# zhang-tao-whu/DVIS_Plus

Hardware: AMD Instinct MI355X
Metric: frames/sec DVIS++ R50 offline, 720p T=30 synthetic (higher is better)
Workload: dtype f32 (storage, accumulation, results; the segmenter's dense layers - R50 convolutions from 128 channels on, pixel-decoder projections and FPN output convolution, the deformable encoder's projections and FFN, the decoder's key / value projections - multiply each fp32 operand as two f16 terms on the f1

## Files before the change

dvis_plus_amd/csrc/gemm.hip:

```cpp
#include "dvis_common.h"

namespace {

constexpr unsigned kOOB = 0x80000000u;

struct GemmArgs {
  const float *A, *W, *bias, *res;
  float *C;
  long long lda, ldw, ldres, ldc;
  long long sA, sW, sRes, sC, sBias;
  int M, N, K, act, row_blocks, col_blocks, vec_store, col_fastest;
};

template <int TILES> constexpr int kGemmMinWaves = TILES >= 32 ? 1 : (TILES >= 20 ? 2 : (TILES >= 12 ? 3 : 4));

template <int RT, int CT, int NW, int PF, bool K16>
__global__ __launch_bounds__(64 * NW, kGemmMinWaves<RT * CT>) void gemm_nt_kernel(const GemmArgs p) {
  extern __shared__ float lds[];
  constexpr int BM = 16 * RT, BN = 16 * CT, T = 64 * NW;

  const int tid = threadIdx.x, lane = tid & 63;
  const int wv = __builtin_amdgcn_readfirstlane(tid >> 6);
  const int i = lane & 15, g = lane >> 4;
  int rb, cb;
  if (p.col_fastest) {
    const unsigned tiles = gridDim.x, xcd = blockIdx.x & 7u, slot = blockIdx.x >> 3;
    const unsigned q8 = tiles >> 3, r8 = tiles & 7u;
    const unsigned logical = (xcd < r8 ? xcd * (q8 + 1) : r8 * (q8 + 1) + (xcd - r8) * q8) + slot;
    rb = (int)(logical / (unsigned)p.col_blocks), cb = (int)(logical % (unsigned)p.col_blocks);
  } else {
    rb = blockIdx.x % p.row_blocks, cb = blockIdx.x / p.row_blocks;
  }
  const int row0 = rb * BM, col0 = cb * BN;
  const long long batch = blockIdx.y;

  const int rows_a = min(BM, p.M - row0), rows_w = min(BN, p.N - col0);
  const float *Ab = p.A + batch * p.sA + (long long)row0 * p.lda;
  const float *Wb = p.W + batch * p.sW + (long long)col0 * p.ldw;
  const __amdgpu_buffer_rsrc_t ra = dvis_make_rsrc_uniform(Ab, (unsigned)((((long long)rows_a - 1) * p.lda + p.K) * 4));
  const __amdgpu_buffer_rsrc_t rw = dvis_make_rsrc_uniform(Wb, (unsigned)((((long long)rows_w - 1) * p.ldw + p.K) * 4));
  unsigned aoff[RT], woff[CT];
#pragma unroll
  for (int rt = 0; rt < RT; ++rt) aoff[rt] = (unsigned)((rt * 16 + i) * p.lda * 4 + g * 16);
#pragma unroll
  for (int ct = 0; ct < CT; ++ct) woff[ct] = (unsigned)((ct * 16 + i) * p.ldw * 4 + g * 16);

  const int G = (p.K + 15) >> 4;
  const int g0 = (int)((long long)G * wv / NW), g1 = (int)((long long)G * (wv + 1) / NW);

  dvis_f4 a[PF][RT], w[PF][CT];
  auto load = [&](int slot, int grp) {
    const bool in = grp < g1;
    const unsigned so = in ? (unsigned)grp * 64u : 0u;
    const bool kv = in && (K16 || grp * 16 + g * 4 < p.K);
#pragma unroll
    for (int rt = 0; rt < RT; ++rt)
      a[slot][rt] = __builtin_bit_cast(
          dvis_f4, __builtin_amdgcn_raw_buffer_load_b128(ra, kv ? aoff[rt] : kOOB, so, 0));
#pragma unroll
    for (int ct = 0; ct < CT; ++ct)
      w[slot][ct] = __builtin_bit_cast(
          dvis_f4, __builtin_amdgcn_raw_buffer_load_b128(rw, kv ? woff[ct] : kOOB, so, 0));
  };

  dvis_f4 acc[RT][CT];
#pragma unroll
  for (int rt = 0; rt < RT; ++rt)
#pragma unroll
    for (int ct = 0; ct < CT; ++ct) acc[rt][ct] = dvis_f4{0.f, 0.f, 0.f, 0.f};

  auto contract = [&](int s) {
#pragma unroll
    for (int c = 0; c < 4; ++c)
#pragma unroll
      for (int rt = 0; rt < RT; ++rt)
#pragma unroll
        for (int ct = 0; ct < CT; ++ct)
          acc[rt][ct] = __builtin_amdgcn_mfma_f32_16x16x4f32(a[s][rt][c], w[s][ct][c], acc[rt][ct], 0, 0, 0);
  };
#pragma unroll
  for (int s = 0; s < PF; ++s) load(s, g0 + s);
  int grp = g0;
#pragma unroll 1
  for (; grp + 2 * PF <= g1; grp += PF) {
#pragma unroll
    for (int s = 0; s < PF; ++s) {
      contract(s);
      __builtin_amdgcn_sched_barrier(0);
      load(s, grp + s + PF);
      __builtin_amdgcn_sched_barrier(0);
    }
  }
  if (grp + PF <= g1) {
#pragma unroll
    for (int s = 0; s < PF; ++s) {
      contract(s);
      if (grp + s + PF < g1) load(s, grp + s + PF);
    }
    grp += PF;
  }
#pragma unroll
  for (int s = 0; s < PF; ++s)
    if (grp + s < g1) contract(s);

  float *mine = lds + wv * (BM * BN);
#pragma unroll
  for (int rt = 0; rt < RT; ++rt)
#pragma unroll
    for (int ct = 0; ct < CT; ++ct)
#pragma unroll
      for (int r = 0; r < 4; ++r) mine[(rt * 16 + g * 4 + r) * BN + ct * 16 + i] = acc[rt][ct][r];
  __syncthreads();

  constexpr int U = BM * BN / 4, UR = BN / 4;
  float *Cb = p.C + batch * p.sC;
  const float *Rb = p.res ? p.res + batch * p.sRes : nullptr;
  const float *Bb = p.bias ? p.bias + batch * p.sBias : nullptr;
#pragma unroll
  for (int u0 = 0; u0 < U; u0 += T) {
    const int u = u0 + tid;
    if (U % T != 0 && u >= U) break;
    const int row = u / UR, c4 = (u - row * UR) * 4;
    dvis_f4 s = *reinterpret_cast<const dvis_f4 *>(lds + row * BN + c4);
#pragma unroll
    for (int k = 1; k < NW; ++k) {
      const dvis_f4 t = *reinterpret_cast<const dvis_f4 *>(lds + k * (BM * BN) + row * BN + c4);
      s = dvis_f4{s[0] + t[0], s[1] + t[1], s[2] + t[2], s[3] + t[3]};
    }
    const int gr = row0 + row, gc = col0 + c4;
    if (gr >= p.M || gc >= p.N) continue;
    float *dst = Cb + (long long)gr * p.ldc + gc;
    if (p.vec_store) {
      if (Bb) {
        const dvis_f4 b = *reinterpret_cast<const dvis_f4 *>(Bb + gc);
        s = dvis_f4{s[0] + b[0], s[1] + b[1], s[2] + b[2], s[3] + b[3]};
      }
      if (Rb) {
        const dvis_f4 t = *reinterpret_cast<const dvis_f4 *>(Rb + (long long)gr * p.ldres + gc);
        s = dvis_f4{s[0] + t[0], s[1] + t[1], s[2] + t[2], s[3] + t[3]};
      }
      if (p.act) s = dvis_f4{fmaxf(s[0], 0.f), fmaxf(s[1], 0.f), fmaxf(s[2], 0.f), fmaxf(s[3], 0.f)};
      *reinterpret_cast<dvis_f4 *>(dst) = s;
    } else {
#pragma unroll
      for (int e = 0; e < 4; ++e) {
        if (gc + e >= p.N) break;
        float v = s[e];
        if (Bb) v += Bb[gc + e];
        if (Rb) v += Rb[(long long)gr * p.ldres + gc + e];
        if (p.act) v = fmaxf(v, 0.f);
        dst[e] = v;
      }
    }
  }
}

template <int RT, int CT, int PF, bool K16>
__global__ __launch_bounds__(64, kGemmMinWaves<RT * CT>) void gemm_nt_persist_kernel(const GemmArgs p) {
  extern __shared__ float lds[];
  constexpr int BM = 16 * RT, BN = 16 * CT, T = 64;
  const int tid = threadIdx.x, lane = tid;
  const int i = lane & 15, g = lane >> 4;
  const long long total = (long long)p.row_blocks * p.col_blocks;
  const unsigned gsz = gridDim.x;
  long long t = (long long)(blockIdx.x & 7u) * (gsz >> 3) + (blockIdx.x >> 3);
  const long long batch = blockIdx.y;
  const float *A0 = p.A + batch * p.sA, *W0 = p.W + batch * p.sW;
  unsigned aoff[RT], woff[CT];
#pragma unroll
  for (int rt = 0; rt < RT; ++rt) aoff[rt] = (unsigned)((rt * 16 + i) * p.lda * 4 + g * 16);
#pragma unroll
  for (int ct = 0; ct < CT; ++ct) woff[ct] = (unsigned)((ct * 16 + i) * p.ldw * 4 + g * 16);
  const int g1 = (p.K + 15) >> 4;

  int row0 = (int)(t / p.col_blocks) * BM, col0 = (int)(t % p.col_blocks) * BN;
  auto desc_a = [&](int r0) {
    const int rows = min(BM, p.M - r0);
    return dvis_make_rsrc_uniform(A0 + (long long)r0 * p.lda, (unsigned)((((long long)rows - 1) * p.lda + p.K) * 4));
  };
  auto desc_w = [&](int c0) {
    const int rows = min(BN, p.N - c0);
    return dvis_make_rsrc_uniform(W0 + (long long)c0 * p.ldw, (unsigned)((((long long)rows - 1) * p.ldw + p.K) * 4));
  };
  __amdgpu_buffer_rsrc_t ra = desc_a(row0), rw = desc_w(col0);

  dvis_f4 a[PF][RT], w[PF][CT];
  auto load = [&](int slot, int grp) {
    const bool in = grp < g1;
    const unsigned so = in ? (unsigned)grp * 64u : 0u;
    const bool kv = in && (K16 || grp * 16 + g * 4 < p.K);
#pragma unroll
    for (int rt = 0; rt < RT; ++rt)
      a[slot][rt] = __builtin_bit_cast(dvis_f4, __builtin_amdgcn_raw_buffer_load_b128(ra, kv ? aoff[rt] : kOOB, so, 0));
#pragma unroll
    for (int ct = 0; ct < CT; ++ct)
      w[slot][ct] = __builtin_bit_cast(dvis_f4, __builtin_amdgcn_raw_buffer_load_b128(rw, kv ? woff[ct] : kOOB, so, 0));
  };
  dvis_f4 acc[RT][CT];
  auto contract = [&](int s) {
#pragma unroll
    for (int c = 0; c < 4; ++c)
#pragma unroll
      for (int rt = 0; rt < RT; ++rt)
#pragma unroll
        for (int ct = 0; ct < CT; ++ct)
          acc[rt][ct] = __builtin_amdgcn_mfma_f32_16x16x4f32(a[s][rt][c], w[s][ct][c], acc[rt][ct], 0, 0, 0);
  };
#pragma unroll
  for (int s = 0; s < PF; ++s) load(s, s);

  float *Cb = p.C + batch * p.sC;
  const float *Rb = p.res ? p.res + batch * p.sRes : nullptr;
  const __amdgpu_buffer_rsrc_t rbias =
      dvis_make_rsrc_uniform(p.bias ? p.bias + batch * p.sBias : p.A, p.bias ? (unsigned)p.N * 4u : 0u);
#pragma unroll 1
  for (;;) {
#pragma unroll
    for (int rt = 0; rt < RT; ++rt)
#pragma unroll
      for (int ct = 0; ct < CT; ++ct) acc[rt][ct] = dvis_f4{0.f, 0.f, 0.f, 0.f};
    int grp = 0;
    auto round = [&]() {
#pragma unroll
      for (int s = 0; s < PF; ++s) {
        contract(s);
        __builtin_amdgcn_sched_barrier(0);
        load(s, grp + s + PF);
        __builtin_amdgcn_sched_barrier(0);
      }
      grp += PF;
    };
    if (grp + 2 * PF <= g1) round();
#pragma unroll 1
    while (grp + 2 * PF <= g1) round();
    if (grp + PF <= g1) {
#pragma unroll
      for (int s = 0; s < PF; ++s) {
        contract(s);
        if (grp + s + PF < g1) load(s, grp + s + PF);
      }
      grp += PF;
    }
#pragma unroll
    for (int s = 0; s < PF; ++s)
      if (grp + s < g1) contract(s);

    const long long tn = t + gsz;
    const bool more = tn < total;
    const int row_e = row0, col_e = col0;
    static_assert(T % (BN / 4) == 0, "a thread keeps its column quad over the epilogue's rounds");
    const int c4_mine = (tid % (BN / 4)) * 4;
    const dvis_f4 bias4 = __builtin_bit_cast(
        dvis_f4, __builtin_amdgcn_raw_buffer_load_b128(rbias, (unsigned)(col_e + c4_mine) * 4u, 0, 0));
    if (more) {
      row0 = (int)(tn / p.col_blocks) * BM, col0 = (int)(tn % p.col_blocks) * BN;
      ra = desc_a(row0), rw = desc_w(col0);
#pragma unroll
      for (int s = 0; s < PF; ++s) load(s, s);
    }
    __syncthreads();
#pragma unroll
    for (int rt = 0; rt < RT; ++rt)
#pragma unroll
      for (int ct = 0; ct < CT; ++ct)
#pragma unroll
        for (int r = 0; r < 4; ++r) lds[(rt * 16 + g * 4 + r) * BN + ct * 16 + i] = acc[rt][ct][r];
    __syncthreads();
    constexpr int U = BM * BN / 4, UR = BN / 4;
#pragma unroll 4
    for (int u = tid; u < U; u += T) {
      const int row = u / UR, c4 = (u - row * UR) * 4;
      dvis_f4 sv = *reinterpret_cast<const dvis_f4 *>(lds + row * BN + c4);
      const int gr = row_e + row, gc = col_e + c4;
      if (gr >= p.M || gc >= p.N) continue;
      float *dst = Cb + (long long)gr * p.ldc + gc;
      if (p.vec_store) {
        sv = dvis_f4{sv[0] + bias4[0], sv[1] + bias4[1], sv[2] + bias4[2], sv[3] + bias4[3]};
        if (Rb) {
          const dvis_f4 tq = *reinterpret_cast<const dvis_f4 *>(Rb + (long long)gr * p.ldres + gc);
          sv = dvis_f4{sv[0] + tq[0], sv[1] + tq[1], sv[2] + tq[2], sv[3] + tq[3]};
        }
        if (p.act) sv = dvis_f4{fmaxf(sv[0], 0.f), fmaxf(sv[1], 0.f), fmaxf(sv[2], 0.f), fmaxf(sv[3], 0.f)};
        *reinterpret_cast<dvis_f4 *>(dst) = sv;
      } else {
#pragma unroll
        for (int e = 0; e < 4; ++e) {
          if (gc + e >= p.N) break;
          float v = sv[e] + bias4[e];
          if (Rb) v += Rb[(long long)gr * p.ldres + gc + e];
          if (p.act) v = fmaxf(v, 0.f);
          dst[e] = v;
        }
      }
    }
    if (!more) break;
    t = tn;
  }
}

struct Config {
  int rt, ct, nw;
  void (*kernel16)(const GemmArgs);
  void (*kernel4)(const GemmArgs);
  void (*persist16)(const GemmArgs);
  void (*persist4)(const GemmArgs);
};
template <int RT, int CT, int NW, int PF, bool K16> constexpr auto persist_or_null() -> void (*)(const GemmArgs) {
  if constexpr (NW == 1) return gemm_nt_persist_kernel<RT, CT, PF, K16>;
  else return nullptr;
}

#define DVIS_GEMM_CFG(RT_, CT_, NW_, PF_)                                                                      \
  { RT_, CT_, NW_, gemm_nt_kernel<RT_, CT_, NW_, PF_, true>, gemm_nt_kernel<RT_, CT_, NW_, PF_, false>,            \
    persist_or_null<RT_, CT_, NW_, PF_, true>(), persist_or_null<RT_, CT_, NW_, PF_, false>() }
const Config kConfigs[] = {
    DVIS_GEMM_CFG(1, 1, 4, 4),
    DVIS_GEMM_CFG(1, 1, 8, 4),
    DVIS_GEMM_CFG(2, 1, 8, 4),
    DVIS_GEMM_CFG(2, 2, 4, 4),
    DVIS_GEMM_CFG(2, 2, 8, 2),
    DVIS_GEMM_CFG(4, 1, 8, 4),
    DVIS_GEMM_CFG(4, 2, 4, 2),
    DVIS_GEMM_CFG(4, 2, 8, 2),
    DVIS_GEMM_CFG(4, 4, 4, 2),
    DVIS_GEMM_CFG(4, 4, 2, 2),
    DVIS_GEMM_CFG(7, 1, 8, 2),
    DVIS_GEMM_CFG(7, 2, 4, 2),
    DVIS_GEMM_CFG(4, 4, 1, 2),
    DVIS_GEMM_CFG(8, 4, 2, 2),
    DVIS_GEMM_CFG(8, 4, 1, 2),
    DVIS_GEMM_CFG(6, 4, 1, 2),
    DVIS_GEMM_CFG(5, 4, 1, 2),
};
constexpr int kNumConfigs = sizeof(kConfigs) / sizeof(kConfigs[0]);

int pick_config(int M, int N, int K, int batch) {
  auto wgs = [&](int c) {
    const long long rb = (M + 16 * kConfigs[c].rt - 1) / (16 * kConfigs[c].rt);
    const long long cb = (N + 16 * kConfigs[c].ct - 1) / (16 * kConfigs[c].ct);
    return rb * cb * batch;
  };
  if ((long long)M * K * 4 > (64ll << 20) && N >= 64) return 14;
  if (wgs(8) >= 256 || (K >= 1024 && wgs(8) >= 128)) return 8;
  if (wgs(6) >= 256) return 6;
  if (wgs(3) >= 192) return K >= 1024 ? 4 : 3;
  if (wgs(2) >= 96) return 2;
  return K >= 256 ? 1 : 0;
}

int pick_config_nw(int M, int N, int K, int batch, int nw) {
  auto wgs = [&](int c) {
    const long long rb = (M + 16 * kConfigs[c].rt - 1) / (16 * kConfigs[c].rt);
    const long long cb = (N + 16 * kConfigs[c].ct - 1) / (16 * kConfigs[c].ct);
    return rb * cb * batch;
  };
  if (nw == 1) return ((long long)M * K * 4 > (64ll << 20) && N >= 64) || wgs(14) >= 1024 ? 14 : 12;
  if (nw == 4) {
    if (wgs(8) >= 256 || (K >= 1024 && wgs(8) >= 128)) return 8;
    if (wgs(6) >= 256) return 6;
    if (wgs(3) >= 192) return 3;
    return 0;
  }
  if (wgs(7) >= 256) return 7;
  if (wgs(4) >= 192) return 4;
  if (wgs(2) >= 96) return 2;
  return 1;
}

}

DVIS_EXPORT int dvis_gemm_num_configs(void) { return kNumConfigs; }

DVIS_EXPORT int dvis_gemm_pick_config_nw(int M, int N, int K, int batch, int nw) {
  if (nw != 1 && nw != 4 && nw != 8) return -1;
  return pick_config_nw(M, N, K, batch > 0 ? batch : 1, nw);
}

DVIS_EXPORT int dvis_gemm_config_waves(int config) { return config >= 0 && config < kNumConfigs ? kConfigs[config].nw : -1; }

DVIS_EXPORT int dvis_gemm_pick_config(int M, int N, int K, int batch) { return pick_config(M, N, K, batch > 0 ? batch : 1); }

static int gemm_launch(const float *A, int64_t lda, int64_t strideA, const float *W, int64_t ldw, int64_t strideW,
                       const float *bias, int64_t strideBias, const float *res, int64_t ldres, int64_t strideRes, float *C,
                       int64_t ldc, int64_t strideC, int M, int N, int K, int batch, int act, int config, void *stream) {
  DVIS_REQUIRE(M >= 0 && N >= 0 && K > 0 && batch >= 0, "gemm_nt: bad sizes (M=%d N=%d K=%d batch=%d)", M, N, K, batch);
  if (M == 0 || N == 0 || batch == 0) return DVIS_OK;
  DVIS_REQUIRE(A && W && C, "gemm_nt: null pointer");
  DVIS_REQUIRE(K % 4 == 0 && lda % 4 == 0 && ldw % 4 == 0 && strideA % 4 == 0 && strideW % 4 == 0 &&
                   ((uintptr_t)A | (uintptr_t)W) % 16 == 0,
               "gemm_nt: needs K, lda, ldw, batch strides %% 4 == 0 and 16-byte aligned A / W (K=%d lda=%lld ldw=%lld)", K,
               (long long)lda, (long long)ldw);
  DVIS_REQUIRE(lda >= K && ldw >= K && ldc >= N && (!res || ldres >= N),
               "gemm_nt: row strides shorter than the rows");
  DVIS_REQUIRE(batch <= 65535, "gemm_nt: batch <= 65535");
  const int c = config >= 0 ? config : pick_config(M, N, K, batch);
  DVIS_REQUIRE(c < kNumConfigs, "gemm_nt: configuration %d does not exist", c);
  const Config &cf = kConfigs[c];
  const int BM = 16 * cf.rt, BN = 16 * cf.ct;
  DVIS_REQUIRE((long long)BM * lda * 4 < (1ll << 31) && (long long)BN * ldw * 4 < (1ll << 31),
               "gemm_nt: one tile's rows must span less than 2 GiB");
  GemmArgs p;
  p.A = A, p.W = W, p.bias = bias, p.res = res, p.C = C;
  p.lda = lda, p.ldw = ldw, p.ldres = ldres, p.ldc = ldc;
  p.sA = strideA, p.sW = strideW, p.sRes = strideRes, p.sC = strideC, p.sBias = strideBias;
  p.M = M, p.N = N, p.K = K, p.act = act;
  p.row_blocks = (M + BM - 1) / BM;
  p.col_blocks = (N + BN - 1) / BN;
  p.col_fastest = (long long)M * K * 4 > (64ll << 20) && p.col_blocks > 1;
  p.vec_store = N % 4 == 0 && ldc % 4 == 0 && strideC % 4 == 0 && (uintptr_t)C % 16 == 0 &&
                (!bias || ((uintptr_t)bias % 16 == 0 && strideBias % 4 == 0)) &&
                (!res || (ldres % 4 == 0 && strideRes % 4 == 0 && (uintptr_t)res % 16 == 0));
  const long long tiles = (long long)p.row_blocks * p.col_blocks;
  DVIS_REQUIRE(tiles < (1ll << 31), "gemm_nt: too many tiles");
  const size_t lds = (size_t)cf.nw * BM * BN * sizeof(float);
  auto kernel = K % 16 == 0 ? cf.kernel16 : cf.kernel4;
  static DvisLdsOptIn opted[kNumConfigs][2];
  if (const int rc = dvis_lds_opt_in(reinterpret_cast<const void *>(kernel), lds, &opted[c][K % 16 == 0 ? 0 : 1], "gemm_nt"))
    return rc;
  static const bool persist_on = []() { const char *e = getenv("DVIS_GEMM_PERSIST"); return !(e && e[0] == '0'); }();
  auto pk = K % 16 == 0 ? cf.persist16 : cf.persist4;
  if (persist_on && pk != nullptr && p.col_fastest) {
    static int cus = 0;
    if (cus == 0) {
      int dev = 0, n = 0;
      hipGetDevice(&dev);
      cus = hipDeviceGetAttribute(&n, hipDeviceAttributeMultiprocessorCount, dev) == hipSuccess && n > 0 ? n : 256;
    }
    const int tiles_cnt = cf.rt * cf.ct;
    const int occ = tiles_cnt >= 32 ? 1 : (tiles_cnt >= 20 ? 2 : (tiles_cnt >= 12 ? 3 : 4));
    const size_t lds1 = (size_t)BM * BN * sizeof(float);
    long long per_cu = 4ll * occ;
    if ((long long)(160 * 1024 / lds1) < per_cu) per_cu = (long long)(160 * 1024 / lds1);
    long long grid = (long long)cus * per_cu;
    if (grid > tiles) grid = tiles;
    grid &= ~7ll;
    if (grid >= 8) {
      hipLaunchKernelGGL(pk, dim3((unsigned)grid, (unsigned)batch), dim3(64), lds1, (hipStream_t)stream, p);
      return dvis_check_launch("gemm_nt_persist_kernel");
    }
  }
  hipLaunchKernelGGL(kernel, dim3((unsigned)tiles, (unsigned)batch), dim3(64 * cf.nw), lds, (hipStream_t)stream, p);
  return dvis_check_launch("gemm_nt_kernel");
}

DVIS_EXPORT int dvis_gemm_nt(const float *A, int64_t lda, int64_t strideA, const float *W, int64_t ldw, int64_t strideW,
                             const float *bias, const float *res, int64_t ldres, int64_t strideRes, float *C,
                             int64_t ldc, int64_t strideC, int M, int N, int K, int batch, int act, int config,
                             void *stream) {
  return gemm_launch(A, lda, strideA, W, ldw, strideW, bias, 0, res, ldres, strideRes, C, ldc, strideC, M, N, K, batch, act,
                     config, stream);
}

DVIS_EXPORT int dvis_gemm_nt_bb(const float *A, int64_t lda, int64_t strideA, const float *W, int64_t ldw, int64_t strideW,
                                const float *bias, int64_t strideBias, const float *res, int64_t ldres, int64_t strideRes,
                                float *C, int64_t ldc, int64_t strideC, int M, int N, int K, int batch, int act, int config,
                                void *stream) {
  return gemm_launch(A, lda, strideA, W, ldw, strideW, bias, strideBias, res, ldres, strideRes, C, ldc, strideC, M, N, K,
                     batch, act, config, stream);
}
```

dvis_plus_amd/csrc/postprocess.hip:

```cpp
#include <math.h>

#include "dvis_common.h"
#include "torch_cpu_math.h"

namespace {

constexpr int kMaxK = 256;
using tcpu::Geometry;
using tcpu::Tap;

__global__ __launch_bounds__(256) void vps_argmax_kernel(
    const float *__restrict__ logits, int64_t stride_k, int64_t stride_t, const float *__restrict__ scores, int K, int T,
    int h, int w, int first_h, int first_w, int img_h, int img_w, int out_h, int out_w, int *__restrict__ ids,
    uint8_t *__restrict__ conf, int *__restrict__ areas ) {
  __shared__ int s_area[3 * kMaxK];
  for (int i = threadIdx.x; i < 3 * K; i += 256) s_area[i] = 0;
  __syncthreads();

  const size_t npix = (size_t)T * out_h * out_w;
  const Geometry g(h, w, first_h, first_w, img_h, img_w, out_h, out_w);
  const int lane = threadIdx.x & 63;
  for (size_t base = (size_t)blockIdx.x * 256; base < npix; base += (size_t)gridDim.x * 256) {
    const size_t p = base + threadIdx.x;
    const bool valid = p < npix;
    const size_t pc = valid ? p : npix - 1;
    const int X = (int)(pc % out_w);
    const size_t r = pc / out_w;
    const int Y = (int)(r % out_h);
    const int t = (int)(r / out_h);
    const Tap ty = tcpu::make_tap(Y, g.s2y, img_h, out_h), tx = tcpu::make_tap(X, g.s2x, img_w, out_w);
    const int kind1 = tcpu::bilinear_kind(first_h, first_w, t, T), kind2 = tcpu::bilinear_kind(out_h, out_w, t, T);
    float best = -INFINITY, best_prob = 0.f;
    int best_k = 0;
    for (int k = 0; k < K; ++k) {
      const float *lg = logits + (size_t)k * stride_k + (size_t)t * stride_t;
      const float prob = tcpu::two_stage<true>(lg, g, Y, X, ty, tx, kind1, kind2);
      const unsigned long long over = __ballot(valid && prob >= 0.5f);
      if (lane == 0 && over) atomicAdd(&s_area[K + k], __popcll(over));
      const float sc = scores[k] * prob;
      if (sc > best) {
        best = sc;
        best_k = k;
        best_prob = prob;
      }
    }
    if (valid) {
      const bool cf = best_prob >= 0.5f;
      ids[p] = best_k;
      conf[p] = cf ? 1 : 0;
      atomicAdd(&s_area[best_k], 1);
      if (cf) atomicAdd(&s_area[2 * K + best_k], 1);
    }
  }
  __syncthreads();
  for (int i = threadIdx.x; i < 3 * K; i += 256)
    if (s_area[i]) atomicAdd(&areas[i], s_area[i]);
}

template <int K4>
__global__ __launch_bounds__(256) void vss_argmax_kernel(
    const float *__restrict__ logits, int64_t stride_q, int64_t stride_t, const float *__restrict__ cls, int Q, int C, int T,
    int h, int w, int first_h, int first_w, int img_h, int img_w, int out_h, int out_w, int64_t *__restrict__ out) {
  const size_t npix = (size_t)T * out_h * out_w;
  const Geometry g(h, w, first_h, first_w, img_h, img_w, out_h, out_w);
  const bool identity2 = img_h == out_h && img_w == out_w;
  for (size_t base = (size_t)blockIdx.x * 256; base < npix; base += (size_t)gridDim.x * 256) {
    const size_t p = base + threadIdx.x;
    const bool valid = p < npix;
    const size_t pc = valid ? p : npix - 1;
    const int X = (int)(pc % out_w);
    const size_t r = pc / out_w;
    const int Y = (int)(r % out_h);
    const int t = (int)(r / out_h);
    const Tap ty = tcpu::make_tap(Y, g.s2y, img_h, out_h), tx = tcpu::make_tap(X, g.s2x, img_w, out_w);
    const int kind1 = tcpu::bilinear_kind(first_h, first_w, t, T), kind2 = tcpu::bilinear_kind(out_h, out_w, t, T);
    float4 acc[K4];
#pragma unroll
    for (int k = 0; k < K4; ++k) acc[k] = make_float4(0.f, 0.f, 0.f, 0.f);
    auto accumulate = [&](int q, float prob) {
      const float4 *row = reinterpret_cast<const float4 *>(cls + (size_t)q * 4 * K4);
#pragma unroll
      for (int k = 0; k < K4; ++k) {
        const float4 cv = row[k];
        acc[k].x += cv.x * prob; acc[k].y += cv.y * prob; acc[k].z += cv.z * prob; acc[k].w += cv.w * prob;
      }
    };
    if (identity2) {
      const Tap sy = tcpu::make_tap(Y, g.s1y, h, first_h), sx = tcpu::make_tap(X, g.s1x, w, first_w);
      const int o00 = sy.i0 * w + sx.i0, o01 = sy.i0 * w + sx.i1, o10 = sy.i1 * w + sx.i0, o11 = sy.i1 * w + sx.i1;
      const float *lg = logits + (size_t)t * stride_t;
      const bool tail = X >= g.tail_x;
      float a = lg[o00], b = lg[o01], c = lg[o10], d = lg[o11];
#pragma unroll 1
      for (int q = 0; q < Q; ++q) {
        const float v = tcpu::bilinear(a, b, c, d, sy, sx, kind1);
        if (q + 1 < Q) {
          const float *nx = lg + (size_t)(q + 1) * stride_q;
          a = nx[o00]; b = nx[o01]; c = nx[o10]; d = nx[o11];
        }
        accumulate(q, tcpu::sigmoid(v, tail));
      }
    } else {
#pragma unroll 1
      for (int q = 0; q < Q; ++q) {
        const float *lg = logits + (size_t)q * stride_q + (size_t)t * stride_t;
        accumulate(q, tcpu::two_stage<true>(lg, g, Y, X, ty, tx, kind1, kind2));
      }
    }
    float best = -INFINITY;
    int best_c = 0;
#pragma unroll
    for (int k = 0; k < K4; ++k) {
      if (4 * k < C && acc[k].x > best) { best = acc[k].x; best_c = 4 * k; }
      if (4 * k + 1 < C && acc[k].y > best) { best = acc[k].y; best_c = 4 * k + 1; }
      if (4 * k + 2 < C && acc[k].z > best) { best = acc[k].z; best_c = 4 * k + 2; }
      if (4 * k + 3 < C && acc[k].w > best) { best = acc[k].w; best_c = 4 * k + 3; }
    }
    if (valid) out[p] = best_c;
  }
}

__global__ __launch_bounds__(256) void vss_argmax_mfma_kernel(
    const float *__restrict__ logits, int64_t stride_q, int64_t stride_t, const float *__restrict__ cls ,
    int Q, int Qp, int C, int T, int h, int w, int first_h, int first_w, int out_h, int out_w, int64_t *__restrict__ out) {
  extern __shared__ __attribute__((aligned(16))) float s_cls[];
  constexpr int LSC = 132;
  constexpr int NT = 2;
  for (int i = threadIdx.x; i < Qp * 128; i += 256) s_cls[(i >> 7) * LSC + (i & 127)] = cls[i];
  __syncthreads();
  const int lane = threadIdx.x & 63, wv = threadIdx.x >> 6;
  const int j = lane & 15, gq = lane >> 4;
  const size_t npix = (size_t)T * out_h * out_w;
  const Geometry g(h, w, first_h, first_w, out_h, out_w, out_h, out_w);
  const size_t nchunks = (npix + 16 * NT - 1) / (16 * NT);
  for (size_t chunk = (size_t)blockIdx.x * 4 + wv; chunk < nchunks; chunk += (size_t)gridDim.x * 4) {
    const float *l00[NT], *l01[NT], *l10[NT], *l11[NT];
    Tap ty1[NT], tx1[NT];
    int kind1[NT];
    bool tail[NT];
#pragma unroll
    for (int n = 0; n < NT; ++n) {
      const size_t p = min(chunk * (16 * NT) + (size_t)n * 16 + j, npix - 1);
      const int X = (int)(p % out_w);
      const size_t r = p / out_w;
      const int Y = (int)(r % out_h);
      const Tap sy = tcpu::make_tap(Y, g.s1y, h, first_h), sx = tcpu::make_tap(X, g.s1x, w, first_w);
      const float *base = logits + (size_t)(r / out_h) * stride_t + (size_t)gq * stride_q;
      l00[n] = base + sy.i0 * w + sx.i0; l01[n] = base + sy.i0 * w + sx.i1;
      l10[n] = base + sy.i1 * w + sx.i0; l11[n] = base + sy.i1 * w + sx.i1;
      ty1[n] = sy; tx1[n] = sx;
      kind1[n] = tcpu::bilinear_kind(first_h, first_w, (int)(r / out_h), T);
      tail[n] = X >= g.tail_x;
    }
    dvis_f4 acc[8][NT];
#pragma unroll
    for (int mt = 0; mt < 8; ++mt)
#pragma unroll
      for (int n = 0; n < NT; ++n) acc[mt][n] = dvis_f4{0.f, 0.f, 0.f, 0.f};
    float va[NT], vb[NT], vc[NT], vd[NT];
    const size_t step = (size_t)4 * stride_q;
#pragma unroll
    for (int n = 0; n < NT; ++n) { va[n] = *l00[n]; vb[n] = *l01[n]; vc[n] = *l10[n]; vd[n] = *l11[n]; }
#pragma unroll 1
    for (int ks = 0; ks < Qp; ks += 4) {
      float pb[NT];
#pragma unroll
      for (int n = 0; n < NT; ++n) {
        pb[n] = tcpu::sigmoid(tcpu::bilinear(va[n], vb[n], vc[n], vd[n], ty1[n], tx1[n], kind1[n]), tail[n]);
      }
      if (ks + 4 < Qp) {
#pragma unroll
        for (int n = 0; n < NT; ++n) {
          l00[n] += step; l01[n] += step; l10[n] += step; l11[n] += step;
          va[n] = *l00[n]; vb[n] = *l01[n]; vc[n] = *l10[n]; vd[n] = *l11[n];
        }
      }
      const float *arow = s_cls + (size_t)(ks + gq) * LSC + j;
#pragma unroll
      for (int mt = 0; mt < 8; ++mt) {
        const float a = arow[16 * mt];
#pragma unroll
        for (int n = 0; n < NT; ++n) acc[mt][n] = __builtin_amdgcn_mfma_f32_16x16x4f32(a, pb[n], acc[mt][n], 0, 0, 0);
      }
    }
#pragma unroll
    for (int n = 0; n < NT; ++n) {
      float best = -INFINITY;
      int best_c = 0x7fffffff;
#pragma unroll
      for (int mt = 0; mt < 8; ++mt)
#pragma unroll
        for (int r = 0; r < 4; ++r) {
          const int c = 16 * mt + 4 * gq + r;
          const float v = acc[mt][n][r];
          if (c < C && v > best) { best = v; best_c = c; }
        }
#pragma unroll
      for (int o = 16; o <= 32; o <<= 1) {
        const float ov = __shfl_xor(best, o);
        const int oc = __shfl_xor(best_c, o);
        if (ov > best || (ov == best && oc < best_c)) { best = ov; best_c = oc; }
      }
      const size_t p = chunk * (16 * NT) + (size_t)n * 16 + j;
      if (gq == 0 && p < npix) out[p] = best_c;
    }
  }
}

__global__ __launch_bounds__(256) void resize2_gt0_kernel(
    const float *__restrict__ logits, int64_t stride_k, int64_t stride_t, int K, int T, int h, int w, int first_h,
    int first_w, int img_h, int img_w, int out_h, int out_w, uint8_t *__restrict__ out) {
  const Geometry g(h, w, first_h, first_w, img_h, img_w, out_h, out_w);
  const int wq = (out_w + 3) >> 2;
  const size_t ngroups = (size_t)K * T * out_h * wq;
  const bool word_ok = (out_w & 3) == 0;
  for (size_t gi = (size_t)blockIdx.x * 256 + threadIdx.x; gi < ngroups; gi += (size_t)gridDim.x * 256) {
    const int xg = (int)(gi % wq);
    size_t r = gi / wq;
    const int Y = (int)(r % out_h);
    r /= out_h;
    const int t = (int)(r % T);
    const int k = (int)(r / T);
    const float *lg = logits + (size_t)k * stride_k + (size_t)t * stride_t;
    const Tap ty = tcpu::make_tap(Y, g.s2y, img_h, out_h);
    const int kind1 = tcpu::bilinear_kind(first_h, first_w, t, T), kind2 = tcpu::bilinear_kind(out_h, out_w, t, T);
    uint8_t *orow = out + (((size_t)k * T + t) * out_h + Y) * out_w;
    unsigned word = 0;
#pragma unroll
    for (int i = 0; i < 4; ++i) {
      const int X = 4 * xg + i;
      if (X < out_w) {
        const Tap tx = tcpu::make_tap(X, g.s2x, img_w, out_w);
        const bool on = tcpu::two_stage<false>(lg, g, Y, X, ty, tx, kind1, kind2) > 0.f;
        if (word_ok) word |= (on ? 1u : 0u) << (8 * i);
        else orow[X] = on ? 1 : 0;
      }
    }
    if (word_ok) *reinterpret_cast<unsigned *>(orow + 4 * xg) = word;
  }
}

template <bool SIGMOID>
__global__ __launch_bounds__(256) void resize2_kernel(
    const float *__restrict__ logits, int64_t stride_k, int64_t stride_t, int K, int T, int h, int w, int first_h,
    int first_w, int img_h, int img_w, int out_h, int out_w, float *__restrict__ out) {
  const Geometry g(h, w, first_h, first_w, img_h, img_w, out_h, out_w);
  const size_t npix = (size_t)K * T * out_h * out_w;
  for (size_t p = (size_t)blockIdx.x * 256 + threadIdx.x; p < npix; p += (size_t)gridDim.x * 256) {
    const int X = (int)(p % out_w);
    size_t r = p / out_w;
    const int Y = (int)(r % out_h);
    r /= out_h;
    const int t = (int)(r % T);
    const int k = (int)(r / T);
    const Tap ty = tcpu::make_tap(Y, g.s2y, img_h, out_h), tx = tcpu::make_tap(X, g.s2x, img_w, out_w);
    const int kind1 = tcpu::bilinear_kind(first_h, first_w, t, T), kind2 = tcpu::bilinear_kind(out_h, out_w, t, T);
    out[p] = tcpu::two_stage<SIGMOID>(logits + (size_t)k * stride_k + (size_t)t * stride_t, g, Y, X, ty, tx, kind1, kind2);
  }
}

}

DVIS_EXPORT int dvis_vps_argmax(const float *logits, int64_t stride_k, int64_t stride_t, const float *scores, int K, int T,
                                int h, int w, int first_h, int first_w, int img_h, int img_w, int out_h, int out_w,
                                int32_t *ids, uint8_t *conf, int32_t *areas, void *stream) {
  DVIS_REQUIRE(K > 0 && K <= kMaxK && T >= 0 && h > 0 && w > 0 && first_h > 0 && first_w > 0 && img_h > 0 && img_w > 0 &&
                   out_h > 0 && out_w > 0,
               "vps_argmax: bad sizes (K must be 1..%d)", kMaxK);
  DVIS_REQUIRE(img_h <= first_h && img_w <= first_w, "vps_argmax: image size exceeds the padded size");
  DVIS_REQUIRE((size_t)T * out_h * out_w < 0x7fffffffu, "vps_argmax: more than 2^31 output pixels");
  DVIS_REQUIRE(logits && scores && ids && conf && areas, "vps_argmax: null pointer");
  hipStream_t st = (hipStream_t)stream;
  if (const int rc = dvis_zero_words(areas, (size_t)3 * K, st, "vps_argmax: zero areas")) return rc;
  if (T == 0) return DVIS_OK;
  const size_t npix = (size_t)T * out_h * out_w;
  size_t blocks = (npix + 255) / 256;
  if (blocks > 256 * 16) blocks = 256 * 16;
  hipLaunchKernelGGL(vps_argmax_kernel, dim3((unsigned)blocks), dim3(256), 0, st, logits, stride_k, stride_t, scores, K, T,
                     h, w, first_h, first_w, img_h, img_w, out_h, out_w, ids, conf, areas);
  return dvis_check_launch("vps_argmax_kernel");
}

DVIS_EXPORT int dvis_vss_argmax(const float *logits, int64_t stride_q, int64_t stride_t, const float *cls,
                                int cls_row_stride, int Q, int C, int T, int h, int w, int first_h, int first_w, int img_h, int img_w, int out_h, int out_w,
                                int64_t *out, void *stream) {
  DVIS_REQUIRE(Q > 0 && C > 0 && C <= 128 && T >= 0 && h > 0 && w > 0 && first_h > 0 && first_w > 0 && img_h > 0 &&
                   img_w > 0 && out_h > 0 && out_w > 0,
               "vss_argmax: bad sizes (C must be 1..128)");
  DVIS_REQUIRE(img_h <= first_h && img_w <= first_w, "vss_argmax: image size exceeds the padded size");
  DVIS_REQUIRE(logits && cls && out, "vss_argmax: null pointer");
  if (T == 0) return DVIS_OK;
  DVIS_REQUIRE(cls_row_stride >= C && cls_row_stride % 32 == 0 && cls_row_stride <= 128 && (((uintptr_t)cls) & 15) == 0,
               "vss_argmax: cls rows must be zero padded to a multiple of 32 floats (<= 128), 16-byte aligned");
  const int k4 = cls_row_stride / 4;
  hipStream_t st = (hipStream_t)stream;
  const size_t npix = (size_t)T * out_h * out_w;
  size_t blocks = (npix + 255) / 256;
  if (img_h == out_h && img_w == out_w && cls_row_stride == 128 && Q % 4 == 0) {
    const size_t lds = (size_t)Q * 132 * sizeof(float);
    if (lds <= 64 * 1024) {
      size_t nb = ((npix + 31) / 32 + 3) / 4;
      if (nb > 256 * 9) nb = 256 * 9;
      hipLaunchKernelGGL(vss_argmax_mfma_kernel, dim3((unsigned)nb), dim3(256), lds, st, logits, stride_q, stride_t, cls, Q, Q,
                         C, T, h, w, first_h, first_w, out_h, out_w, out);
      return dvis_check_launch("vss_argmax_mfma_kernel");
    }
  }
  if (blocks > 256 * 16) blocks = 256 * 16;
#define DVIS_VSS(K4_)                                                                                                   \
  hipLaunchKernelGGL((vss_argmax_kernel<K4_>), dim3((unsigned)blocks), dim3(256), 0, st, logits, stride_q, stride_t, cls, \
                     Q, C, T, h, w, first_h, first_w, img_h, img_w, out_h, out_w, out)
  if (k4 == 8) DVIS_VSS(8);
  else if (k4 == 16) DVIS_VSS(16);
  else if (k4 == 24) DVIS_VSS(24);
  else DVIS_VSS(32);
#undef DVIS_VSS
  return dvis_check_launch("vss_argmax_kernel");
}

DVIS_EXPORT int dvis_resize2_gt0(const float *logits, int64_t stride_k, int64_t stride_t, int K, int T, int h, int w,
                                 int first_h, int first_w, int img_h, int img_w, int out_h, int out_w, uint8_t *out,
                                 void *stream) {
  DVIS_REQUIRE(K >= 0 && T >= 0 && h > 0 && w > 0 && first_h > 0 && first_w > 0 && img_h > 0 && img_w > 0 && out_h > 0 &&
                   out_w > 0,
               "resize2_gt0: bad sizes");
  DVIS_REQUIRE(img_h <= first_h && img_w <= first_w, "resize2_gt0: image size exceeds the padded size");
  if (K == 0 || T == 0) return DVIS_OK;
  DVIS_REQUIRE(logits && out, "resize2_gt0: null pointer");
  DVIS_REQUIRE((((uintptr_t)out) & 3) == 0, "resize2_gt0: out must be 4-byte aligned");
  const size_t ngroups = (size_t)K * T * out_h * ((out_w + 3) / 4);
  size_t blocks = (ngroups + 255) / 256;
  if (blocks > 256 * 64) blocks = 256 * 64;
  hipLaunchKernelGGL(resize2_gt0_kernel, dim3((unsigned)blocks), dim3(256), 0, (hipStream_t)stream, logits, stride_k,
                     stride_t, K, T, h, w, first_h, first_w, img_h, img_w, out_h, out_w, out);
  return dvis_check_launch("resize2_gt0_kernel");
}

DVIS_EXPORT int dvis_resize2(const float *logits, int64_t stride_k, int64_t stride_t, int K, int T, int h, int w,
                             int first_h, int first_w, int img_h, int img_w, int out_h, int out_w, int sigmoid, float *out,
                             void *stream) {
  DVIS_REQUIRE(K >= 0 && T >= 0 && h > 0 && w > 0 && first_h > 0 && first_w > 0 && img_h > 0 && img_w > 0 && out_h > 0 &&
                   out_w > 0,
               "resize2: bad sizes");
  DVIS_REQUIRE(img_h <= first_h && img_w <= first_w, "resize2: image size exceeds the padded size");
  if (K == 0 || T == 0) return DVIS_OK;
  DVIS_REQUIRE(logits && out, "resize2: null pointer");
  const size_t npix = (size_t)K * T * out_h * out_w;
  size_t blocks = (npix + 255) / 256;
  if (blocks > 256 * 64) blocks = 256 * 64;
  if (sigmoid)
    hipLaunchKernelGGL(resize2_kernel<true>, dim3((unsigned)blocks), dim3(256), 0, (hipStream_t)stream, logits, stride_k,
                       stride_t, K, T, h, w, first_h, first_w, img_h, img_w, out_h, out_w, out);
  else
    hipLaunchKernelGGL(resize2_kernel<false>, dim3((unsigned)blocks), dim3(256), 0, (hipStream_t)stream, logits, stride_k,
                       stride_t, K, T, h, w, first_h, first_w, img_h, img_w, out_h, out_w, out);
  return dvis_check_launch("resize2_kernel");
}
```

dvis_plus_amd/csrc/torch_cpu_math.h:

```cpp
#pragma once
#include <hip/hip_runtime.h>

namespace tcpu {

struct Tap {
  int i0, i1;
  float l0, l1;
};

__device__ __forceinline__ Tap make_tap(int dst, float scale, int in, int out) {
#pragma clang fp contract(off)
  Tap t;
  if (in == out) {
    t.i0 = t.i1 = dst;
    t.l0 = 1.f;
    t.l1 = 0.f;
    return t;
  }
  float src = __builtin_fmaf(scale, (float)dst + 0.5f, -0.5f);
  src = src < 0.f ? 0.f : src;
  t.i0 = min((int)src, in - 1);
  t.i1 = t.i0 + (t.i0 < in - 1 ? 1 : 0);
  t.l1 = fminf(fmaxf(src - (float)t.i0, 0.f), 1.f);
  t.l0 = 1.f - t.l1;
  return t;
}

enum { kGeneric = 0, kSmallTail = 1, kSmallVec = 2 };

__device__ __forceinline__ int bilinear_kind(int out_h, int out_w, int channel, int channels) {
  if (out_h + out_w > 128) return kGeneric;
  return channel < (channels & ~15) ? kSmallVec : kSmallTail;
}

__device__ __forceinline__ float bilinear(float a, float b, float c, float d, const Tap &ty, const Tap &tx, int kind) {
#pragma clang fp contract(off)
  if (kind == kGeneric) {
    const float tA = __builtin_fmaf(a, tx.l0, b * tx.l1);
    const float tB = __builtin_fmaf(c, tx.l0, d * tx.l1);
    return __builtin_fmaf(tA, ty.l0, tB * ty.l1);
  }
  const float w00 = ty.l0 * tx.l0, w01 = ty.l0 * tx.l1, w10 = ty.l1 * tx.l0, w11 = ty.l1 * tx.l1;
  if (kind == kSmallVec) return __builtin_fmaf(w00, a, __builtin_fmaf(w01, b, __builtin_fmaf(w11, d, w10 * c)));
  return __builtin_fmaf(w11, d, __builtin_fmaf(w10, c, __builtin_fmaf(w00, a, w01 * b)));
}

__device__ __forceinline__ float sleef_expf(float d) {
#pragma clang fp contract(off)
  const float R_LN2f = 1.442695040888963407359924681001892137426645954152985934135449406931f;
  const float L2Uf = 0.693145751953125f, L2Lf = 1.428606765330187045e-06f;
  const float qf = rintf(d * R_LN2f);
  const int q = (int)qf;
  float s = __builtin_fmaf(qf, -L2Uf, d);
  s = __builtin_fmaf(qf, -L2Lf, s);
  float u = 0.000198527617612853646278381f;
  u = __builtin_fmaf(u, s, 0.00139304355252534151077271f);
  u = __builtin_fmaf(u, s, 0.00833336077630519866943359f);
  u = __builtin_fmaf(u, s, 0.0416664853692054748535156f);
  u = __builtin_fmaf(u, s, 0.166666671633720397949219f);
  u = __builtin_fmaf(u, s, 0.5f);
  u = 1.0f + __builtin_fmaf(s * s, u, s);
  const int q1 = q >> 1, q2 = q - q1;
  u = u * __int_as_float((q1 + 127) << 23);
  u = u * __int_as_float((q2 + 127) << 23);
  if (d < -104.f) u = 0.f;
  if (d > 100.f) u = INFINITY;
  return u;
}

__device__ __forceinline__ float sigmoid(float x, bool scalar_tail) {
#pragma clang fp contract(off)
  const float nx = 0.f - x;
  const float e = scalar_tail ? (float)exp((double)nx) : sleef_expf(nx);
  return 1.f / (1.f + e);
}

struct Geometry {
  int h, w, first_h, first_w, img_h, img_w, out_h, out_w;
  float s1y, s1x, s2y, s2x;
  int tail_x;
  __device__ __forceinline__ Geometry(int h_, int w_, int fh, int fw, int ih, int iw, int oh, int ow)
      : h(h_), w(w_), first_h(fh), first_w(fw), img_h(ih), img_w(iw), out_h(oh), out_w(ow) {
    s1y = (float)h / (float)first_h;
    s1x = (float)w / (float)first_w;
    s2y = (float)img_h / (float)out_h;
    s2x = (float)img_w / (float)out_w;
    tail_x = img_w != first_w ? (img_w & ~31) : 0x7fffffff;
  }
};

template <bool SIGMOID>
__device__ __forceinline__ float stage1(const float *__restrict__ lg, const Geometry &g, int yy, int xx, int kind1) {
  const Tap ty = make_tap(yy, g.s1y, g.h, g.first_h), tx = make_tap(xx, g.s1x, g.w, g.first_w);
  const float a = lg[ty.i0 * g.w + tx.i0], b = lg[ty.i0 * g.w + tx.i1];
  const float c = lg[ty.i1 * g.w + tx.i0], d = lg[ty.i1 * g.w + tx.i1];
  const float v = bilinear(a, b, c, d, ty, tx, kind1);
  return SIGMOID ? sigmoid(v, xx >= g.tail_x) : v;
}

template <bool SIGMOID>
__device__ __forceinline__ float two_stage(const float *__restrict__ lg, const Geometry &g, int Y, int X, const Tap &ty2,
                                           const Tap &tx2, int kind1, int kind2) {
  if (g.img_h == g.out_h && g.img_w == g.out_w) return stage1<SIGMOID>(lg, g, Y, X, kind1);
  const float a = stage1<SIGMOID>(lg, g, ty2.i0, tx2.i0, kind1), b = stage1<SIGMOID>(lg, g, ty2.i0, tx2.i1, kind1);
  const float c = stage1<SIGMOID>(lg, g, ty2.i1, tx2.i0, kind1), d = stage1<SIGMOID>(lg, g, ty2.i1, tx2.i1, kind1);
  return bilinear(a, b, c, d, ty2, tx2, kind2);
}

}
```

Baseline: 409.3.

## Split-K GEMM reduction by owner wave; hoist taps and prefetch in argmax postprocess

The multi-wave GEMM epilogue previously had every wave dump its full accumulator tile to LDS and then summed across waves. Now each wave owns a slice of the output elements: the other waves write only that slice into its LDS region, and the owner reduces it and stores its own results. This cuts LDS footprint and traffic. Separately, the VPS argmax kernel precomputes bilinear site offsets and taps once per pixel rather than per query, software-prefetches the next query's four logits through 32-bit-offset buffer loads, and batches per-query area counts into one atomic per 64 queries. This adds complexity and new LDS-layout indexing that could be wrong.

```diff
diff --git a/dvis_plus_amd/csrc/gemm.hip b/dvis_plus_amd/csrc/gemm.hip
--- a/dvis_plus_amd/csrc/gemm.hip
+++ b/dvis_plus_amd/csrc/gemm.hip
@@ -103,32 +103,12 @@
   for (int s = 0; s < PF; ++s)
     if (grp + s < g1) contract(s);
 
-  float *mine = lds + wv * (BM * BN);
-#pragma unroll
-  for (int rt = 0; rt < RT; ++rt)
-#pragma unroll
-    for (int ct = 0; ct < CT; ++ct)
-#pragma unroll
-      for (int r = 0; r < 4; ++r) mine[(rt * 16 + g * 4 + r) * BN + ct * 16 + i] = acc[rt][ct][r];
-  __syncthreads();
-
-  constexpr int U = BM * BN / 4, UR = BN / 4;
   float *Cb = p.C + batch * p.sC;
   const float *Rb = p.res ? p.res + batch * p.sRes : nullptr;
   const float *Bb = p.bias ? p.bias + batch * p.sBias : nullptr;
-#pragma unroll
-  for (int u0 = 0; u0 < U; u0 += T) {
-    const int u = u0 + tid;
-    if (U % T != 0 && u >= U) break;
-    const int row = u / UR, c4 = (u - row * UR) * 4;
-    dvis_f4 s = *reinterpret_cast<const dvis_f4 *>(lds + row * BN + c4);
-#pragma unroll
-    for (int k = 1; k < NW; ++k) {
-      const dvis_f4 t = *reinterpret_cast<const dvis_f4 *>(lds + k * (BM * BN) + row * BN + c4);
-      s = dvis_f4{s[0] + t[0], s[1] + t[1], s[2] + t[2], s[3] + t[3]};
-    }
+  auto finish = [&](dvis_f4 s, int row, int c4) {
     const int gr = row0 + row, gc = col0 + c4;
-    if (gr >= p.M || gc >= p.N) continue;
+    if (gr >= p.M || gc >= p.N) return;
     float *dst = Cb + (long long)gr * p.ldc + gc;
     if (p.vec_store) {
       if (Bb) {
@@ -150,6 +130,70 @@
         if (Rb) v += Rb[(long long)gr * p.ldres + gc + e];
         if (p.act) v = fmaxf(v, 0.f);
         dst[e] = v;
+      }
+    }
+  };
+
+  if constexpr (NW == 1) {
+#pragma unroll
+    for (int rt = 0; rt < RT; ++rt)
+#pragma unroll
+      for (int ct = 0; ct < CT; ++ct)
+#pragma unroll
+        for (int r = 0; r < 4; ++r) lds[(rt * 16 + g * 4 + r) * BN + ct * 16 + i] = acc[rt][ct][r];
+    __syncthreads();
+    constexpr int U = BM * BN / 4, UR = BN / 4;
+#pragma unroll
+    for (int u0 = 0; u0 < U; u0 += T) {
+      const int u = u0 + tid;
+      if (U % T != 0 && u >= U) break;
+      const int row = u / UR, c4 = (u - row * UR) * 4;
+      finish(*reinterpret_cast<const dvis_f4 *>(lds + row * BN + c4), row, c4);
+    }
+  } else {
+    constexpr int NP = RT * CT * 4, PO = (NP + NW - 1) / NW, NO = NP < NW ? NP : NW;
+    constexpr int SLOT = PO * 64, REGION = (NW - 1) * SLOT;
+#pragma unroll
+    for (int o = 0; o < NO; ++o) {
+      if (o != wv) {
+        float *dst = lds + o * REGION + (wv < o ? wv : wv - 1) * SLOT + lane;
+#pragma unroll
+        for (int q = o; q < NP; q += NW) dst[(q / NW) * 64] = acc[(q >> 2) / CT][(q >> 2) % CT][q & 3];
+      }
+    }
+    __syncthreads();
+#pragma unroll
+    for (int o = 0; o < NO; ++o) {
+      if (o == wv) {
+        float *reg = lds + o * REGION + lane;
+#pragma unroll
+        for (int q = o; q < NP; q += NW) {
+          const int j = q / NW;
+          const float own = acc[(q >> 2) / CT][(q >> 2) % CT][q & 3];
+          float s = o == 0 ? own : reg[j * 64];
+#pragma unroll
+          for (int k = 1; k < NW; ++k) {
+            const float t = k == o ? own : reg[(k < o ? k : k - 1) * SLOT + j * 64];
+            s = s + t;
+          }
+          reg[j * 64] = s;
+        }
+      }
+    }
+    if (wv < NO) {
+      __builtin_amdgcn_fence(__ATOMIC_RELEASE, "wavefront");
+      __builtin_amdgcn_wave_barrier();
+      __builtin_amdgcn_fence(__ATOMIC_ACQUIRE, "wavefront");
+      const int units = ((NP - wv + NW - 1) / NW) * 16;
+      const float *reg = lds + wv * REGION;
+#pragma unroll
+      for (int u0 = 0; u0 < PO * 16; u0 += 64) {
+        const int u = u0 + lane;
+        if (u < units) {
+          const int q = wv + (u >> 4) * NW, tile = q >> 2;
+          finish(*reinterpret_cast<const dvis_f4 *>(reg + u * 4), (tile / CT) * 16 + ((u >> 2) & 3) * 4 + (q & 3),
+                 (tile % CT) * 16 + (u & 3) * 4);
+        }
       }
     }
   }
@@ -296,6 +340,12 @@
     if (!more) break;
     t = tn;
   }
+}
+
+size_t gemm_nt_lds_bytes(int rt, int ct, int nw) {
+  if (nw == 1) return (size_t)256 * rt * ct * sizeof(float);
+  const int np = 4 * rt * ct, po = (np + nw - 1) / nw, no = np < nw ? np : nw;
+  return (size_t)no * (nw - 1) * po * 64 * sizeof(float);
 }
 
 struct Config {
@@ -412,7 +462,7 @@
                 (!res || (ldres % 4 == 0 && strideRes % 4 == 0 && (uintptr_t)res % 16 == 0));
   const long long tiles = (long long)p.row_blocks * p.col_blocks;
   DVIS_REQUIRE(tiles < (1ll << 31), "gemm_nt: too many tiles");
-  const size_t lds = (size_t)cf.nw * BM * BN * sizeof(float);
+  const size_t lds = gemm_nt_lds_bytes(cf.rt, cf.ct, cf.nw);
   auto kernel = K % 16 == 0 ? cf.kernel16 : cf.kernel4;
   static DvisLdsOptIn opted[kNumConfigs][2];
   if (const int rc = dvis_lds_opt_in(reinterpret_cast<const void *>(kernel), lds, &opted[c][K % 16 == 0 ? 0 : 1], "gemm_nt"))
diff --git a/dvis_plus_amd/csrc/postprocess.hip b/dvis_plus_amd/csrc/postprocess.hip
--- a/dvis_plus_amd/csrc/postprocess.hip
+++ b/dvis_plus_amd/csrc/postprocess.hip
@@ -8,6 +8,138 @@
 constexpr int kMaxK = 256;
 using tcpu::Geometry;
 using tcpu::Tap;
+
+struct NarrowMaps {
+  using Off = unsigned;
+  __amdgpu_buffer_rsrc_t rs;
+  __device__ __forceinline__ NarrowMaps(const float *base, unsigned bytes) : rs(dvis_make_rsrc_uniform(base, bytes)) {}
+  __device__ __forceinline__ float operator()(Off o) const {
+    return __builtin_bit_cast(float, __builtin_amdgcn_raw_buffer_load_b32(rs, o, 0, 0));
+  }
+};
+struct WideMaps {
+  using Off = long long;
+  const float *base;
+  __device__ __forceinline__ WideMaps(const float *base_, unsigned) : base(base_) {}
+  __device__ __forceinline__ float operator()(Off o) const {
+    return *reinterpret_cast<const float *>(reinterpret_cast<const char *>(base) + o);
+  }
+};
+template <typename OffT>
+struct SiteOffsets {
+  OffT o[4];
+};
+template <typename OffT>
+__device__ __forceinline__ SiteOffsets<OffT> site_offsets(const tcpu::Stage1Site &s, long long frame) {
+  SiteOffsets<OffT> r;
+  r.o[0] = (OffT)((frame + s.o00) * 4), r.o[1] = (OffT)((frame + s.o01) * 4);
+  r.o[2] = (OffT)((frame + s.o10) * 4), r.o[3] = (OffT)((frame + s.o11) * 4);
+  return r;
+}
+
+template <typename Maps>
+__device__ __forceinline__ void vps_argmax_body(
+    const float *__restrict__ logits, int64_t stride_k, int64_t stride_t, const float *__restrict__ scores, int K, int T,
+    int h, int w, int first_h, int first_w, int img_h, int img_w, int out_h, int out_w, int *__restrict__ ids,
+    uint8_t *__restrict__ conf, int *s_area, unsigned map_bytes) {
+  using OffT = typename Maps::Off;
+  const unsigned npix = (unsigned)T * out_h * out_w;
+  const Geometry g(h, w, first_h, first_w, img_h, img_w, out_h, out_w);
+  const bool identity2 = img_h == out_h && img_w == out_w;
+  const int lane = threadIdx.x & 63;
+  for (unsigned base = blockIdx.x * 256u; base < npix; base += gridDim.x * 256u) {
+    const unsigned p = base + threadIdx.x;
+    const bool valid = p < npix;
+    const unsigned pc = valid ? p : npix - 1;
+    const int X = (int)(pc % (unsigned)out_w);
+    const unsigned r = pc / (unsigned)out_w;
+    const int Y = (int)(r % (unsigned)out_h);
+    const int t = (int)(r / (unsigned)out_h);
+    const int kind1 = tcpu::bilinear_kind(first_h, first_w, t, T), kind2 = tcpu::bilinear_kind(out_h, out_w, t, T);
+    const long long frame = (long long)t * stride_t;
+    float best = -INFINITY, best_prob = 0.f;
+    int best_k = 0;
+    auto take = [&](int k, float score, float prob, int &cnt) {
+      const unsigned long long over = __builtin_amdgcn_ballot_w64(valid && prob >= 0.5f);
+      cnt += lane == (k & 63) ? __popcll(over) : 0;
+      const float sc = score * prob;
+      if (sc > best) {
+        best = sc;
+        best_k = k;
+        best_prob = prob;
+      }
+    };
+    auto flush = [&](int k0, int cnt) {
+      if (cnt) atomicAdd(&s_area[K + k0 + lane], cnt);
+    };
+    float score = scores[0];
+    if (identity2) {
+      const tcpu::Stage1Site s = tcpu::make_stage1_site(g, Y, X);
+      const SiteOffsets<OffT> so = site_offsets<OffT>(s, frame);
+      const Maps m0(logits, map_bytes);
+      float a = m0(so.o[0]), b = m0(so.o[1]), c = m0(so.o[2]), d = m0(so.o[3]);
+      for (int k0 = 0; k0 < K; k0 += 64) {
+        const int k1 = min(k0 + 64, K);
+        int cnt = 0;
+#pragma unroll 1
+        for (int k = k0; k < k1; ++k) {
+          const float v = tcpu::stage1_value(a, b, c, d, s, kind1);
+          const float sk = score;
+          if (k + 1 < K) {
+            const Maps nx(logits + (size_t)(k + 1) * stride_k, map_bytes);
+            a = nx(so.o[0]), b = nx(so.o[1]), c = nx(so.o[2]), d = nx(so.o[3]);
+            score = scores[k + 1];
+          }
+          take(k, sk, tcpu::sigmoid(v, s.tail), cnt);
+        }
+        flush(k0, cnt);
+      }
+    } else {
+      const Tap ty = tcpu::make_tap(Y, g.s2y, img_h, out_h), tx = tcpu::make_tap(X, g.s2x, img_w, out_w);
+      const tcpu::Stage1Site s[4] = {tcpu::make_stage1_site(g, ty.i0, tx.i0), tcpu::make_stage1_site(g, ty.i0, tx.i1),
+                                     tcpu::make_stage1_site(g, ty.i1, tx.i0), tcpu::make_stage1_site(g, ty.i1, tx.i1)};
+      SiteOffsets<OffT> so[4];
+      float v[4][4];
+      const Maps m0(logits, map_bytes);
+#pragma unroll
+      for (int j = 0; j < 4; ++j) {
+        so[j] = site_offsets<OffT>(s[j], frame);
+#pragma unroll
+        for (int e = 0; e < 4; ++e) v[j][e] = m0(so[j].o[e]);
+      }
+      for (int k0 = 0; k0 < K; k0 += 64) {
+        const int k1 = min(k0 + 64, K);
+        int cnt = 0;
+#pragma unroll 1
+        for (int k = k0; k < k1; ++k) {
+          float f[4];
+#pragma unroll
+          for (int j = 0; j < 4; ++j) f[j] = tcpu::stage1_value(v[j][0], v[j][1], v[j][2], v[j][3], s[j], kind1);
+          const float sk = score;
+          if (k + 1 < K) {
+            const Maps nx(logits + (size_t)(k + 1) * stride_k, map_bytes);
+#pragma unroll
+            for (int j = 0; j < 4; ++j)
+#pragma unroll
+              for (int e = 0; e < 4; ++e) v[j][e] = nx(so[j].o[e]);
+            score = scores[k + 1];
+          }
+#pragma unroll
+          for (int j = 0; j < 4; ++j) f[j] = tcpu::sigmoid(f[j], s[j].tail);
+          take(k, sk, tcpu::bilinear(f[0], f[1], f[2], f[3], ty, tx, kind2), cnt);
+        }
+        flush(k0, cnt);
+      }
+    }
+    if (valid) {
+      const bool cf = best_prob >= 0.5f;
+      ids[p] = best_k;
+      conf[p] = cf ? 1 : 0;
+      atomicAdd(&s_area[best_k], 1);
+      if (cf) atomicAdd(&s_area[2 * K + best_k], 1);
+    }
+  }
+}
 
 __global__ __launch_bounds__(256) void vps_argmax_kernel(
     const float *__restrict__ logits, int64_t stride_k, int64_t stride_t, const float *__restrict__ scores, int K, int T,
@@ -17,41 +149,13 @@
   for (int i = threadIdx.x; i < 3 * K; i += 256) s_area[i] = 0;
   __syncthreads();
 
-  const size_t npix = (size_t)T * out_h * out_w;
-  const Geometry g(h, w, first_h, first_w, img_h, img_w, out_h, out_w);
-  const int lane = threadIdx.x & 63;
-  for (size_t base = (size_t)blockIdx.x * 256; base < npix; base += (size_t)gridDim.x * 256) {
-    const size_t p = base + threadIdx.x;
-    const bool valid = p < npix;
-    const size_t pc = valid ? p : npix - 1;
-    const int X = (int)(pc % out_w);
-    const size_t r = pc / out_w;
-    const int Y = (int)(r % out_h);
-    const int t = (int)(r / out_h);
-    const Tap ty = tcpu::make_tap(Y, g.s2y, img_h, out_h), tx = tcpu::make_tap(X, g.s2x, img_w, out_w);
-    const int kind1 = tcpu::bilinear_kind(first_h, first_w, t, T), kind2 = tcpu::bilinear_kind(out_h, out_w, t, T);
-    float best = -INFINITY, best_prob = 0.f;
-    int best_k = 0;
-    for (int k = 0; k < K; ++k) {
-      const float *lg = logits + (size_t)k * stride_k + (size_t)t * stride_t;
-      const float prob = tcpu::two_stage<true>(lg, g, Y, X, ty, tx, kind1, kind2);
-      const unsigned long long over = __ballot(valid && prob >= 0.5f);
-      if (lane == 0 && over) atomicAdd(&s_area[K + k], __popcll(over));
-      const float sc = scores[k] * prob;
-      if (sc > best) {
-        best = sc;
-        best_k = k;
-        best_prob = prob;
-      }
-    }
-    if (valid) {
-      const bool cf = best_prob >= 0.5f;
-      ids[p] = best_k;
-      conf[p] = cf ? 1 : 0;
-      atomicAdd(&s_area[best_k], 1);
-      if (cf) atomicAdd(&s_area[2 * K + best_k], 1);
-    }
-  }
+  const long long map_bytes = ((long long)(T - 1) * stride_t + (long long)h * w) * 4;
+  if (stride_t >= 0 && map_bytes <= 0xffffffffll)
+    vps_argmax_body<NarrowMaps>(logits, stride_k, stride_t, scores, K, T, h, w, first_h, first_w, img_h, img_w, out_h,
+                                out_w, ids, conf, s_area, (unsigned)map_bytes);
+  else
+    vps_argmax_body<WideMaps>(logits, stride_k, stride_t, scores, K, T, h, w, first_h, first_w, img_h, img_w, out_h,
+                              out_w, ids, conf, s_area, 0u);
   __syncthreads();
   for (int i = threadIdx.x; i < 3 * K; i += 256)
     if (s_area[i]) atomicAdd(&areas[i], s_area[i]);
diff --git a/dvis_plus_amd/csrc/torch_cpu_math.h b/dvis_plus_amd/csrc/torch_cpu_math.h
--- a/dvis_plus_amd/csrc/torch_cpu_math.h
+++ b/dvis_plus_amd/csrc/torch_cpu_math.h
@@ -98,6 +98,26 @@
   return SIGMOID ? sigmoid(v, xx >= g.tail_x) : v;
 }
 
+struct Stage1Site {
+  Tap ty, tx;
+  int o00, o01, o10, o11;
+  bool tail;
+};
+
+__device__ __forceinline__ Stage1Site make_stage1_site(const Geometry &g, int yy, int xx) {
+  Stage1Site s;
+  s.ty = make_tap(yy, g.s1y, g.h, g.first_h);
+  s.tx = make_tap(xx, g.s1x, g.w, g.first_w);
+  s.o00 = s.ty.i0 * g.w + s.tx.i0, s.o01 = s.ty.i0 * g.w + s.tx.i1;
+  s.o10 = s.ty.i1 * g.w + s.tx.i0, s.o11 = s.ty.i1 * g.w + s.tx.i1;
+  s.tail = xx >= g.tail_x;
+  return s;
+}
+
+__device__ __forceinline__ float stage1_value(float a, float b, float c, float d, const Stage1Site &s, int kind1) {
+  return bilinear(a, b, c, d, s.ty, s.tx, kind1);
+}
+
 template <bool SIGMOID>
 __device__ __forceinline__ float two_stage(const float *__restrict__ lg, const Geometry &g, int Y, int X, const Tap &ty2,
                                            const Tap &tx2, int kind1, int kind2) {
```

Result: no change. 405.8 (-0.9%).
